# Hendrik1704/GPBayesTools-HIC

Measured on AMD Instinct MI355X. Metric: MCMC steps/s x walkers (walker log-posterior evaluations per second, whole job), higher is better.
Workload: dtype f64

## Files before the change

### gpbayestools_hic_amd/build.py

```python
import os
import subprocess
import sys

HERE = os.path.dirname(os.path.abspath(__file__))
CSRC = os.path.join(HERE, "csrc")
LIB = os.path.join(HERE, "libgpbayes.so")
LIB_DEBUG = os.path.join(HERE, "libgpbayes_debug.so")
SOURCES = ["gpb_api.hip", "gpb_fit.hip", "gpb_chol.hip", "gpb_predict.hip", "gpb_sliced.hip", "gpb_like.hip", "gpb_cov.hip", "gpb_pmap.hip", "gpb_pool.hip",
           "gpb_grad.hip", "gpb_ptlmc.hip", "gpb_smc.hip", "gpb_cv.hip"]
HEADERS = ["gpb_internal.h", "gemm_tile.h", "chol_block.h", "fast_math.h", "philox.h", os.path.join("..", "..", "include", "gpbayes.h"),
           os.path.join("..", "..", "include", "gpbayes_debug.h")]


def _stale(lib=LIB):
    if not os.path.exists(lib):
        return True
    t = os.path.getmtime(lib)
    return any(os.path.getmtime(os.path.join(CSRC, f)) > t for f in SOURCES + HEADERS)


def build_native(force=False, verbose=False, debug_variants=False):
    lib = LIB_DEBUG if debug_variants else LIB
    if not force and not _stale(lib):
        return lib
    hipcc = os.environ.get("HIPCC", "/opt/rocm/bin/hipcc")
    objs = []
    procs = []
    bdir = os.path.join(HERE, "build", "debug" if debug_variants else "product")
    os.makedirs(bdir, exist_ok=True)
    for src in SOURCES:
        obj = os.path.join(bdir, src.replace(".hip", ".o"))
        cmd = [hipcc, "--offload-arch=gfx950", "-O3", "-std=c++17", "-fPIC", "-fvisibility=hidden", "-c",
               os.path.join(CSRC, src), "-o", obj] + (["-DGPB_DEBUG_VARIANTS"] if debug_variants else [])
        if debug_variants:
            cmd += os.environ.get("GPB_DEBUG_EXTRA_DEFINES", "").split()
        if verbose:
            print(" ".join(cmd), file=sys.stderr)
        procs.append((cmd, subprocess.Popen(cmd, stdout=subprocess.PIPE, stderr=subprocess.STDOUT)))
        objs.append(obj)
    for cmd, p in procs:
        out, _ = p.communicate()
        if p.returncode != 0:
            raise RuntimeError("hipcc failed: %s\n%s" % (" ".join(cmd), out.decode()))
    cmd = [hipcc, "--offload-arch=gfx950", "-shared", "-fPIC", "-Wl,-Bsymbolic", "-o", lib] + objs + ["-ldl"]
    r = subprocess.run(cmd, stdout=subprocess.PIPE, stderr=subprocess.STDOUT)
    if r.returncode != 0:
        raise RuntimeError("link failed: %s\n%s" % (" ".join(cmd), r.stdout.decode()))
    return lib


if __name__ == "__main__":
    print(build_native(force="--force" in sys.argv, verbose=True))
    if "--debug-variants" in sys.argv:
        print(build_native(force="--force" in sys.argv, verbose=True, debug_variants=True))
```

### gpbayestools_hic_amd/csrc/gpb_sliced.hip

```cpp
#include "gpb_internal.h"

namespace gpb {

typedef int v4i __attribute__((ext_vector_type(4)));
typedef int v16i __attribute__((ext_vector_type(16)));
typedef __attribute__((address_space(3))) void* sl_lds_ptr;

template <int D>
struct SlDig {
    static constexpr int LOW = D - 1, NLEV = 2 * D - 1 - LOW, BITS = 8 * D - 1;
    static constexpr unsigned long long HALF = 0x8080808080808080ull >> (64 - 8 * D);
};
constexpr int SL_DMAX = 7;
constexpr int64_t SL_NP_MAX = 16384;
constexpr int SL_BM = 128;
template <int D, int WTN>
struct SlGeo {
    static constexpr int BN = 64 * WTN;
    static constexpr int A_CHUNKS = D * 2 * (SL_BM / 64), B_CHUNKS = D * 2 * WTN, CHUNKS = A_CHUNKS + B_CHUNKS;
    static constexpr int STAGE = CHUNKS * 1024, NSTAGE = 3;
    static constexpr int LDS = NSTAGE * STAGE + SL_BM * 8;
    static constexpr int NPW = (CHUNKS + 7) / 8, REM = CHUNKS % 8;
};
constexpr int SL_RG = 8, SL_CG = 4;
constexpr double SL_RULE = 128.0;

template <int D>
__device__ __forceinline__ unsigned long long sl_digits(long long a) {
    return ((unsigned long long)a + SlDig<D>::HALF) ^ SlDig<D>::HALF;
}

__device__ __forceinline__ int sl_exponent(double m) {
    int ex;
    const double f = frexp(m, &ex);
    return f <= 0.99 ? ex : ex + 1;
}

__global__ __launch_bounds__(256) void k_sl_rowscale(const double* __restrict__ Linv, const double* __restrict__ amp,
                                                     double* __restrict__ rowscale, int* __restrict__ rowexp,
                                                     double* __restrict__ colscale, int64_t Np, int64_t Np128) {
    const int p = blockIdx.y, lane = threadIdx.x & 63;
    const int64_t j = (int64_t)blockIdx.x * 4 + (threadIdx.x >> 6);
    if (j >= Np128) return;
    double m = 0.0;
    if (j < Np) {
        const double* row = Linv + ((int64_t)p * Np + j) * Np;
        for (int64_t k = lane; k <= j; k += 64) m = fmax(m, fabs(row[k]));
#pragma unroll
        for (int o = 32; o > 0; o >>= 1) m = fmax(m, __shfl_xor(m, o));
    }
    if (lane == 0) {
        const int e = m > 0.0 ? sl_exponent(m) : 0;
        rowexp[(int64_t)p * Np128 + j] = e;
        rowscale[(int64_t)p * Np128 + j] = ldexp(1.0, e - 14);
        if (j == 0) colscale[p] = ldexp(1.0, sl_exponent(amp[p]));
    }
}

template <int D>
__global__ __launch_bounds__(256) void k_sl_slice_linv(const double* __restrict__ Linv, const int* __restrict__ rowexp,
                                                       int8_t* __restrict__ planes, int64_t Np, int64_t Np128) {
    const int p = blockIdx.z;
    const int64_t j = (int64_t)blockIdx.x * 256 + threadIdx.x, kb = blockIdx.y;
    if (j >= Np || kb * 16 > j) return;
    const double* src = Linv + ((int64_t)p * Np + j) * Np + kb * 16;
    const int e = rowexp[(int64_t)p * Np128 + j];
    unsigned long long dg[16];
#pragma unroll
    for (int i = 0; i < 16; ++i) {
        const double x = (kb * 16 + i <= j) ? src[i] : 0.0;
        dg[i] = sl_digits<D>(__double2ll_rn(ldexp(x, SlDig<D>::BITS - e)));
    }
    const int64_t plane = (Np / 16) * Np128 * 16;
    int8_t* dst = planes + (int64_t)p * D * plane + (kb * Np128 + j) * 16;
#pragma unroll
    for (int t = 0; t < D; ++t) {
        unsigned w[4];
#pragma unroll
        for (int g = 0; g < 4; ++g)
            w[g] = (unsigned)((dg[4 * g] >> (8 * t)) & 0xff) | (unsigned)(((dg[4 * g + 1] >> (8 * t)) & 0xff) << 8) |
                   (unsigned)(((dg[4 * g + 2] >> (8 * t)) & 0xff) << 16) | (unsigned)(((dg[4 * g + 3] >> (8 * t)) & 0xff) << 24);
        *reinterpret_cast<uint4*>(dst + t * plane) = make_uint4(w[0], w[1], w[2], w[3]);
    }
}


template <int D, int WTN>
__device__ __forceinline__ void sl_dma_stage(char* lds, int buf, const int8_t* __restrict__ Ap, const int8_t* __restrict__ Bp,
                                             int64_t a_plane, int64_t b_plane, int64_t Np128, int64_t Wld, int64_t mb, int64_t nb,
                                             int64_t kb0, int wave, int lane) {
    typedef SlGeo<D, WTN> G;
    char* base = lds + buf * G::STAGE;
#pragma unroll
    for (int c = 0; c < G::NPW; ++c) {
        const int ch = 8 * c + wave;
        if (c == G::NPW - 1 && G::REM != 0 && wave >= G::REM) break;
        const bool is_a = ch < G::A_CHUNKS;
        const int cb = is_a ? ch : ch - G::A_CHUNKS;
        const int per = is_a ? SL_BM / 64 : WTN;
        const int t = cb / (2 * per), q = (cb / per) & 1, h = cb % per;
        const int64_t ld = is_a ? Np128 : Wld, off = is_a ? mb : nb;
        const int8_t* plane = is_a ? Ap + t * a_plane : Bp + t * b_plane;
        const int8_t* src = plane + ((kb0 + q) * ld + off + 64 * h + lane) * 16;
        __builtin_amdgcn_global_load_lds((const void*)src, (sl_lds_ptr)(base + ch * 1024), 16, 0, 0);
    }
}

template <int N>
__device__ __forceinline__ void sl_wait_vm() { asm volatile("s_waitcnt vmcnt(%0)" ::"n"(N) : "memory"); }

template <int D, int WTN>
__device__ __forceinline__ void sl_wait_stage(bool more, bool full_count) {
    typedef SlGeo<D, WTN> G;
    if (!more) sl_wait_vm<0>();
    else if (full_count) sl_wait_vm<G::NPW>();
    else sl_wait_vm<G::NPW - 1>();
}

template <int D, int WTN>
__device__ __forceinline__ void sl_mma_step(const char* lds, int buf, int wm, int wn, int lane, v16i (&acc)[SlDig<D>::NLEV][WTN]) {
    typedef SlGeo<D, WTN> G;
    constexpr int LOW = SlDig<D>::LOW;
    const char* base = lds + buf * G::STAGE;
    const int q = lane >> 5, r = lane & 31;
    v4i a[D];
#pragma unroll
    for (int t = 0; t < D; ++t) a[t] = *reinterpret_cast<const v4i*>(base + ((t * 2 + q) * SL_BM + wm * 32 + r) * 16);
#pragma unroll
    for (int j = 0; j < WTN; ++j) {
        v4i b[D];
#pragma unroll
        for (int t = 0; t < D; ++t)
            b[t] = *reinterpret_cast<const v4i*>(base + G::A_CHUNKS * 1024 + ((t * 2 + q) * G::BN + wn * 32 * WTN + 32 * j + r) * 16);
#pragma unroll
        for (int tb = 0; tb < D; ++tb)
#pragma unroll
            for (int ta = 0; ta < D; ++ta) {
                if (ta + tb < LOW) continue;
                acc[ta + tb - LOW][j] = __builtin_amdgcn_mfma_i32_32x32x32_i8(a[ta], b[tb], acc[ta + tb - LOW][j], 0, 0, 0);
            }
    }
}

struct SlGP {
    const int8_t *A, *B;
    const double *rowscale, *colscale;
    double* spart;
    int P, p;
};
constexpr int SL_MAX_GP = GPB_MAX_MULTI_GP;
struct SlTable { SlGP gp[SL_MAX_GP]; };

template <int D, int WTN, bool MULTI>
__device__ __forceinline__ void predict_sliced_body(const SlGP& G0, const SlTable* __restrict__ tab, int64_t Np, int64_t Np128, int64_t Wld,
                                                    int P, int nI, int nW, int kskip, const int* __restrict__ nrows) {
    typedef SlGeo<D, WTN> G;
    constexpr int NLEV = SlDig<D>::NLEV;
    extern __shared__ __attribute__((aligned(16))) char lds[];
    if (nrows) nW = (*nrows + G::BN - 1) / G::BN;
    const int nG = (nI + SL_RG - 1) / SL_RG, nWG = (nW + SL_CG - 1) / SL_CG;
    const unsigned label = blockIdx.x & 7u, m = blockIdx.x >> 3;
    const unsigned sb = (m / (SL_RG * SL_CG)) * 8u + label, local = m % (SL_RG * SL_CG);
    if (sb >= (unsigned)(nG * P * nWG)) return;
    const int g = (int)(sb / (unsigned)(P * nWG)), rem = (int)(sb % (unsigned)(P * nWG));
    const int pg = rem / nWG, wg = rem % nWG;
    const SlGP gp = MULTI ? tab->gp[pg] : G0;
    const int p = MULTI ? gp.p : pg;
    const int8_t* __restrict__ A = gp.A;
    const int8_t* __restrict__ B = gp.B;
    const double* __restrict__ rowscale = gp.rowscale;
    const double* __restrict__ colscale = gp.colscale;
    double* __restrict__ spart = gp.spart;
    const int Pc = MULTI ? gp.P : P;
    const int ib = (nG - 1 - g) * SL_RG + (SL_RG - 1 - (int)(local / SL_CG)), wt = wg * SL_CG + (int)(local % SL_CG);
    if (ib >= nI || wt >= nW) return;
    const int tid = threadIdx.x, lane = tid & 63;
    const int wave = __builtin_amdgcn_readfirstlane(tid >> 6);
    const int wm = wave >> 1, wn = wave & 1;
    const int64_t mb = (int64_t)ib * SL_BM, nb = (int64_t)wt * G::BN;
    const bool fullc = G::REM == 0 || wave < G::REM;
    const int64_t a_plane = (Np / 16) * Np128 * 16, b_plane = (Np / 16) * Wld * 16;
    const int8_t* Ap = A + (int64_t)p * D * a_plane;
    const int8_t* Bp = B + (int64_t)p * D * b_plane;
    double* rs = reinterpret_cast<double*>(lds + G::NSTAGE * G::STAGE);
    if (tid < SL_BM) rs[tid] = rowscale[(int64_t)p * Np128 + mb + tid];
    const int64_t k_end = imin64(mb + SL_BM, Np);
    const int64_t ks = (kskip / 32) * 32;
    const int64_t k_begin = ks <= mb ? ks : 0;
    const int nsteps = (int)((k_end - k_begin) / 32);
    const int64_t kb_first = k_begin / 16;
    v16i acc[NLEV][WTN];
#pragma unroll
    for (int l = 0; l < NLEV; ++l)
#pragma unroll
        for (int j = 0; j < WTN; ++j)
#pragma unroll
            for (int r = 0; r < 16; ++r) acc[l][j][r] = 0;
    sl_dma_stage<D, WTN>(lds, 0, Ap, Bp, a_plane, b_plane, Np128, Wld, mb, nb, kb_first, wave, lane);
    if (nsteps > 1) sl_dma_stage<D, WTN>(lds, 1, Ap, Bp, a_plane, b_plane, Np128, Wld, mb, nb, kb_first + 2, wave, lane);
    for (int s = 0; s < nsteps; ++s) {
        asm volatile("s_waitcnt lgkmcnt(0)" ::: "memory");
        sl_wait_stage<D, WTN>(s + 1 < nsteps, fullc);
        __builtin_amdgcn_s_barrier();
        sl_mma_step<D, WTN>(lds, s % 3, wm, wn, lane, acc);
        if (s + 2 < nsteps)
            sl_dma_stage<D, WTN>(lds, (s + 2) % 3, Ap, Bp, a_plane, b_plane, Np128, Wld, mb, nb, kb_first + 2 * (int64_t)(s + 2), wave, lane);
    }
    asm volatile("s_waitcnt lgkmcnt(0)" ::: "memory");
    __builtin_amdgcn_s_barrier();
    const double cs = colscale[p];
    double* hand = reinterpret_cast<double*>(lds);
    double sums[WTN];
#pragma unroll
    for (int j = 0; j < WTN; ++j) {
        double sum = 0.0;
#pragma unroll
        for (int r = 0; r < 16; ++r) {
            double t = (double)acc[0][j][r];
#pragma unroll
            for (int l = 1; l < NLEV; ++l) t = fma(t, 1.0 / 256.0, (double)acc[l][j][r]);
            const int row = wm * 32 + (r & 3) + 8 * (r >> 2) + 4 * (lane >> 5);
            const double v = t * rs[row] * cs;
            sum = fma(v, v, sum);
        }
        sum += __shfl_xor(sum, 32);
        sums[j] = sum;
        if ((wm & 1) && lane < 32) hand[(wave * WTN + j) * 32 + lane] = sum;
    }
    __syncthreads();
    const int64_t blk = (int64_t)ib * 2 + (wm >> 1);
    if (!(wm & 1) && lane < 32 && blk * 64 < Np) {
#pragma unroll
        for (int j = 0; j < WTN; ++j)
            spart[(blk * Pc + p) * Wld + nb + wn * 32 * WTN + 32 * j + lane] = sums[j] + hand[((wave + 2) * WTN + j) * 32 + lane];
    }
}

template <int D, int WTN>
__global__ __launch_bounds__(512, 2) void k_predict_sliced(const SlGP gp, int64_t Np, int64_t Np128, int64_t Wld, int P, int nI, int nW,
                                                           int kskip, const int* __restrict__ nrows) {
    predict_sliced_body<D, WTN, false>(gp, nullptr, Np, Np128, Wld, P, nI, nW, kskip, nrows);
}

template <int D, int WTN>
__global__ __launch_bounds__(512, 2) void k_predict_sliced_multi(const SlTable tab, int64_t Np, int64_t Np128, int64_t Wld, int P, int nI,
                                                                 int nW, int kskip, const int* __restrict__ nrows) {
    predict_sliced_body<D, WTN, true>(tab.gp[0], &tab, Np, Np128, Wld, P, nI, nW, kskip, nrows);
}

int sliced_applies(const gpb_ctx* ctx) {
    if (!ctx->predict_sliced || ctx->multi || !ctx->h_theta || !ctx->have_theta) return 0;
    if (ctx->tile_trace) return 0;
    if (ctx->Np > SL_NP_MAX) return 0;
    if (ctx->predict_sliced == 3) return 7;
    if (ctx->predict_sliced == 2) return 6;
    const int64_t stride = ctx->d + 2;
    for (int64_t p = 0; p < ctx->P; ++p) {
        const double lc = ctx->h_theta[p * stride], ln = ctx->h_theta[p * stride + ctx->d + 1];
        if (!(1.0 + exp(lc - ln) <= SL_RULE)) return 0;
    }
    return 6;
}

void sliced_free(gpb_ctx* ctx) {
    if (ctx->slA) { pool_free(ctx->slA); ctx->slA = nullptr; }
    if (ctx->slB) { pool_free(ctx->slB); ctx->slB = nullptr; }
    if (ctx->sl_scale) { pool_free(ctx->sl_scale); ctx->sl_scale = nullptr; }
    ctx->slA_valid = false;
    ctx->slA_depth = 0;
    ctx->slB_cap = 0;
}

const double* sliced_colscale(const gpb_ctx* ctx) {
    return reinterpret_cast<const double*>(ctx->sl_scale) + ctx->P * round_up(ctx->Np, 128);
}

int sliced_prepare(gpb_ctx* ctx, int depth) {
    if (depth != 6 && depth != 7) GPB_FAIL(GPB_E_STATE, "gpb: internal: sliced_prepare at a depth other than 6 or 7");
    const int64_t Np = ctx->Np, Np128 = round_up(Np, 128), P = ctx->P;
    const size_t a_bytes = (size_t)P * SL_DMAX * (size_t)Np * (size_t)Np128;
    if (!ctx->slA) {
        GPB_HIP(pool_malloc_t(&ctx->slA, a_bytes));
        GPB_HIP(hipMemsetAsync(ctx->slA, 0, a_bytes, ctx->stream));
        GPB_HIP(pool_malloc_t(&ctx->sl_scale, sizeof(double) * (size_t)(P * Np128 + P) + sizeof(int) * (size_t)(P * Np128)));
        ctx->slA_valid = false;
    }
    double* rowscale = reinterpret_cast<double*>(ctx->sl_scale);
    double* colscale = rowscale + P * Np128;
    int* rowexp = reinterpret_cast<int*>(colscale + P);
    if (!ctx->slA_valid || ctx->slA_depth != depth) {
        hipLaunchKernelGGL(k_sl_rowscale, dim3((unsigned)((Np128 + 3) / 4), (unsigned)P), dim3(256), 0, ctx->stream, ctx->Linv,
                           ctx->amp, rowscale, rowexp, colscale, Np, Np128);
        const dim3 grid((unsigned)((Np + 255) / 256), (unsigned)(Np / 16), (unsigned)P);
        if (depth == 7)
            hipLaunchKernelGGL(k_sl_slice_linv<7>, grid, dim3(256), 0, ctx->stream, ctx->Linv, rowexp, ctx->slA, Np, Np128);
        else
            hipLaunchKernelGGL(k_sl_slice_linv<6>, grid, dim3(256), 0, ctx->stream, ctx->Linv, rowexp, ctx->slA, Np, Np128);
        ctx->slA_valid = true;
        ctx->slA_depth = depth;
    }
    if (ctx->slB_cap < ctx->Wcap || !ctx->slB) {
        if (ctx->slB) { GPB_HIP(hipStreamSynchronize(ctx->stream)); pool_free(ctx->slB); ctx->slB = nullptr; }
        GPB_HIP(pool_malloc_t(&ctx->slB, (size_t)P * SL_DMAX * (size_t)Np * (size_t)ctx->Wcap));
        ctx->slB_cap = ctx->Wcap;
    }
    GPB_HIP(hipGetLastError());
    return 0;
}

int sliced_read_kstar(gpb_ctx* ctx, int64_t p, int64_t pad, int64_t N, int64_t W, double* out) {
    const int D = ctx->batch_sliced;
    if (D != 6 && D != 7) GPB_FAIL(GPB_E_STATE, "gpb: internal: sliced_read_kstar without a sliced batch");
    const int64_t Np = ctx->Np, Wld = ctx->Wld, plane = (Np / 16) * Wld * 16;
    std::vector<int8_t> h((size_t)(D * plane));
    double cs = 0.0;
    GPB_HIP(hipStreamSynchronize(ctx->stream));
    GPB_HIP(hipMemcpy(h.data(), ctx->slB + p * D * plane, (size_t)(D * plane), hipMemcpyDeviceToHost));
    GPB_HIP(hipMemcpy(&cs, sliced_colscale(ctx) + p, sizeof(double), hipMemcpyDeviceToHost));
    for (int64_t n = 0; n < N; ++n)
        for (int64_t w = 0; w < W; ++w) {
            const int64_t k = pad + n;
            long long a = 0;
            for (int t = D - 1; t >= 0; --t) a = a * 256 + (long long)h[(size_t)(t * plane + ((k / 16) * Wld + w) * 16 + k % 16)];
            out[n * W + w] = ldexp((double)a, -(8 * D - 1)) * cs;
        }
    return 0;
}

static int sliced_wtn(const gpb_ctx* ctx, int depth, int64_t gps, int nI, int64_t W, const int* nrows_dev) {
    if (depth == 7) return 1;
    const int64_t Wsel = imin64(ctx->Wld, live_rows_estimate(ctx, W, nrows_dev, ctx->Wld));
    const int64_t tiles128 = gps * nI * ((Wsel + 127) / 128);
    int wtn = tiles128 >= 3 * (int64_t)ctx->num_cu ? 2 : 1;
    if (ctx->force_tile == 128) wtn = 2;
    if (ctx->force_tile == 64 || ctx->force_tile == 32 || ctx->force_tile == 65) wtn = 1;
    return wtn;
}

template <int D, int WTN, bool MULTI, class Arg>
static int sliced_launch(gpb_ctx* ctx, const Arg& arg, int64_t Np, int64_t Np128, int64_t Wld, int G, int nI, int kskip,
                         const int* nrows_dev) {
    typedef SlGeo<D, WTN> Geo;
    const int nW = (int)(Wld / Geo::BN);
    const int nG = (nI + SL_RG - 1) / SL_RG, nWG = (nW + SL_CG - 1) / SL_CG;
    const int64_t nSB = (int64_t)nG * G * nWG;
    const unsigned grid = (unsigned)(((nSB + 7) / 8) * 8 * SL_RG * SL_CG);
    if constexpr (MULTI) {
        GPB_HIP(hipFuncSetAttribute((const void*)k_predict_sliced_multi<D, WTN>, hipFuncAttributeMaxDynamicSharedMemorySize, Geo::LDS));
        hipLaunchKernelGGL((k_predict_sliced_multi<D, WTN>), dim3(grid), dim3(512), Geo::LDS, ctx->stream, arg, Np, Np128, Wld, G, nI, nW,
                           kskip, nrows_dev);
    } else {
        GPB_HIP(hipFuncSetAttribute((const void*)k_predict_sliced<D, WTN>, hipFuncAttributeMaxDynamicSharedMemorySize, Geo::LDS));
        hipLaunchKernelGGL((k_predict_sliced<D, WTN>), dim3(grid), dim3(512), Geo::LDS, ctx->stream, arg, Np, Np128, Wld, G, nI, nW,
                           kskip, nrows_dev);
    }
    return 0;
}

template <bool MULTI, class Arg>
static int sliced_dispatch(gpb_ctx* ctx, int depth, int wtn, const Arg& arg, int64_t Np, int64_t Np128, int64_t Wld, int G, int nI,
                           int kskip, const int* nrows_dev) {
    if (depth == 7) return sliced_launch<7, 1, MULTI>(ctx, arg, Np, Np128, Wld, G, nI, kskip, nrows_dev);
    if (wtn == 2) return sliced_launch<6, 2, MULTI>(ctx, arg, Np, Np128, Wld, G, nI, kskip, nrows_dev);
    return sliced_launch<6, 1, MULTI>(ctx, arg, Np, Np128, Wld, G, nI, kskip, nrows_dev);
}

int launch_vsq_sliced(gpb_ctx* ctx, int64_t W, const int* nrows_dev, int kskip) {
    const int64_t Np = ctx->Np, Np128 = round_up(Np, 128), P = ctx->P, Wld = ctx->Wld;
    const int depth = ctx->batch_sliced;
    if (!ctx->slA || !ctx->slA_valid || !ctx->slB || ctx->slA_depth != depth)
        GPB_FAIL(GPB_E_STATE, "gpb: internal: launch_vsq_sliced before sliced_prepare");
    const double* rowscale = reinterpret_cast<const double*>(ctx->sl_scale);
    const double* colscale = rowscale + P * Np128;
    const int nI = (int)(Np128 / SL_BM);
    const int wtn = sliced_wtn(ctx, depth, P, nI, W, nrows_dev);
    const SlGP gp{ctx->slA, ctx->slB, rowscale, colscale, ctx->spart, (int)P, 0};
    return sliced_dispatch<false>(ctx, depth, wtn, gp, Np, Np128, Wld, (int)P, nI, kskip, nrows_dev);
}

int launch_vsq_sliced_multi(gpb_ctx* const* ctxs, int E, int64_t W, const int* nrows_dev, int kskip) {
    gpb_ctx* ctx = ctxs[0];
    const int64_t Np = ctx->Np, Np128 = round_up(Np, 128), Wld = ctx->Wld;
    const int depth = ctx->batch_sliced;
    SlTable tab;
    int G = 0;
    for (int e = 0; e < E; ++e) {
        gpb_ctx* c = ctxs[e];
        if (!c->slA || !c->slA_valid || !c->slB || c->Np != Np || c->Wld != Wld || c->batch_sliced != depth || c->slA_depth != depth)
            GPB_FAIL(GPB_E_STATE, "gpb: internal: launch_vsq_sliced_multi over a context that is not prepared");
        const double* rowscale = reinterpret_cast<const double*>(c->sl_scale);
        const double* colscale = rowscale + c->P * Np128;
        for (int p = 0; p < (int)c->P; ++p, ++G) {
            if (G >= SL_MAX_GP) GPB_FAIL(GPB_E_STATE, "gpb: internal: launch_vsq_sliced_multi: too many GPs for one table");
            tab.gp[G] = SlGP{c->slA, c->slB, rowscale, colscale, c->spart, (int)c->P, p};
        }
    }
    const int nI = (int)(Np128 / SL_BM);
    const int wtn = sliced_wtn(ctx, depth, G, nI, W, nrows_dev);
    return sliced_dispatch<true>(ctx, depth, wtn, tab, Np, Np128, Wld, G, nI, kskip, nrows_dev);
}

}
```

Baseline: 1.497 million.

## Ping-pong wave groups between LDS reads and MFMA in sliced GEMM

Replaces the per-step read-then-MFMA loop with a schedule in which two groups of four waves alternate between loading LDS operands and issuing MFMAs. The group offset comes from one extra barrier, so one group's LDS reads overlap the other group's matrix work, and each step is split into per-column sub-steps. The DMA source address is also made wave-uniform through readfirstlane, with the lane offset added afterwards. The cost is roughly twice as many barriers per step plus extra sched_barrier fences that limit compiler reordering.

```diff
diff --git a/gpbayestools_hic_amd/build.py b/gpbayestools_hic_amd/build.py
--- a/gpbayestools_hic_amd/build.py
+++ b/gpbayestools_hic_amd/build.py
@@ -8,7 +8,7 @@
 LIB_DEBUG = os.path.join(HERE, "libgpbayes_debug.so")
 SOURCES = ["gpb_api.hip", "gpb_fit.hip", "gpb_chol.hip", "gpb_predict.hip", "gpb_sliced.hip", "gpb_like.hip", "gpb_cov.hip", "gpb_pmap.hip", "gpb_pool.hip",
            "gpb_grad.hip", "gpb_ptlmc.hip", "gpb_smc.hip", "gpb_cv.hip"]
-HEADERS = ["gpb_internal.h", "gemm_tile.h", "chol_block.h", "fast_math.h", "philox.h", os.path.join("..", "..", "include", "gpbayes.h"),
+HEADERS = ["gpb_internal.h", "gemm_tile.h", "sliced_schedule.h", "chol_block.h", "fast_math.h", "philox.h", os.path.join("..", "..", "include", "gpbayes.h"),
            os.path.join("..", "..", "include", "gpbayes_debug.h")]
 
 
diff --git a/gpbayestools_hic_amd/csrc/gpb_sliced.hip b/gpbayestools_hic_amd/csrc/gpb_sliced.hip
--- a/gpbayestools_hic_amd/csrc/gpb_sliced.hip
+++ b/gpbayestools_hic_amd/csrc/gpb_sliced.hip
@@ -1,4 +1,5 @@
 #include "gpb_internal.h"
+#include "sliced_schedule.h"
 
 namespace gpb {
 
@@ -21,6 +22,8 @@
     static constexpr int STAGE = CHUNKS * 1024, NSTAGE = 3;
     static constexpr int LDS = NSTAGE * STAGE + SL_BM * 8;
     static constexpr int NPW = (CHUNKS + 7) / 8, REM = CHUNKS % 8;
+    static_assert(NSTAGE == SL_SCHED_BUFFERS && CHUNKS == sl_sched_chunks(D, WTN) && NPW == sl_sched_npw(D, WTN) && REM == sl_sched_rem(D, WTN),
+                  "sliced_schedule.h models another geometry");
 };
 constexpr int SL_RG = 8, SL_CG = 4;
 constexpr double SL_RULE = 128.0;
@@ -101,8 +104,10 @@
         const int t = cb / (2 * per), q = (cb / per) & 1, h = cb % per;
         const int64_t ld = is_a ? Np128 : Wld, off = is_a ? mb : nb;
         const int8_t* plane = is_a ? Ap + t * a_plane : Bp + t * b_plane;
-        const int8_t* src = plane + ((kb0 + q) * ld + off + 64 * h + lane) * 16;
-        __builtin_amdgcn_global_load_lds((const void*)src, (sl_lds_ptr)(base + ch * 1024), 16, 0, 0);
+        const uint64_t us = (uint64_t)(plane + ((kb0 + q) * ld + off + 64 * h) * 16);
+        const int8_t* src = (const int8_t*)(((uint64_t)(unsigned)__builtin_amdgcn_readfirstlane((int)(us >> 32)) << 32) |
+                                            (uint64_t)(unsigned)__builtin_amdgcn_readfirstlane((int)us));
+        __builtin_amdgcn_global_load_lds((const void*)(src + (unsigned)(lane << 4)), (sl_lds_ptr)(base + ch * 1024), 16, 0, 0);
     }
 }
 
@@ -118,29 +123,51 @@
 }
 
 template <int D, int WTN>
-__device__ __forceinline__ void sl_mma_step(const char* lds, int buf, int wm, int wn, int lane, v16i (&acc)[SlDig<D>::NLEV][WTN]) {
+struct SlWave {
     typedef SlGeo<D, WTN> G;
-    constexpr int LOW = SlDig<D>::LOW;
-    const char* base = lds + buf * G::STAGE;
-    const int q = lane >> 5, r = lane & 31;
-    v4i a[D];
-#pragma unroll
-    for (int t = 0; t < D; ++t) a[t] = *reinterpret_cast<const v4i*>(base + ((t * 2 + q) * SL_BM + wm * 32 + r) * 16);
-#pragma unroll
-    for (int j = 0; j < WTN; ++j) {
-        v4i b[D];
-#pragma unroll
-        for (int t = 0; t < D; ++t)
-            b[t] = *reinterpret_cast<const v4i*>(base + G::A_CHUNKS * 1024 + ((t * 2 + q) * G::BN + wn * 32 * WTN + 32 * j + r) * 16);
+    static constexpr int NLEV = SlDig<D>::NLEV, LOW = SlDig<D>::LOW;
+    char* lds;
+    const int8_t *Ap, *Bp;
+    int64_t a_plane, b_plane, Np128, Wld, mb, nb, kb_first;
+    int wave, lane, wm, wn;
+    bool fullc;
+    v4i a[D], b[D];
+    v16i acc[NLEV][WTN];
+
+    __device__ __forceinline__ void issue(int stage, int buf) {
+        sl_dma_stage<D, WTN>(lds, buf, Ap, Bp, a_plane, b_plane, Np128, Wld, mb, nb, kb_first + 2 * (int64_t)stage, wave, lane);
+    }
+    template <int J>
+    __device__ __forceinline__ void read(int, int buf) {
+        const int q = lane >> 5, r = lane & 31;
+        const char* pa = lds + (buf * G::STAGE + (q * SL_BM + wm * 32 + r) * 16);
+        const char* pb = lds + (buf * G::STAGE + G::A_CHUNKS * 1024 + (q * G::BN + wn * 32 * WTN + r) * 16);
+#pragma unroll
+        for (int t = 0; t < D; ++t) a[t] = *reinterpret_cast<const v4i*>(pa + t * 2 * SL_BM * 16);
+#pragma unroll
+        for (int t = 0; t < D; ++t) b[t] = *reinterpret_cast<const v4i*>(pb + (t * 2 * G::BN + 32 * J) * 16);
+    }
+    __device__ __forceinline__ void reads_done() { asm volatile("s_waitcnt lgkmcnt(0)" ::: "memory"); }
+    __device__ __forceinline__ void wait(bool newest_flies) {
+        reads_done();
+        sl_wait_stage<D, WTN>(newest_flies, fullc);
+    }
+    __device__ __forceinline__ void barrier() {
+        __builtin_amdgcn_sched_barrier(0);
+        __builtin_amdgcn_s_barrier();
+        __builtin_amdgcn_sched_barrier(0);
+    }
+    template <int J>
+    __device__ __forceinline__ void mma() {
 #pragma unroll
         for (int tb = 0; tb < D; ++tb)
 #pragma unroll
             for (int ta = 0; ta < D; ++ta) {
                 if (ta + tb < LOW) continue;
-                acc[ta + tb - LOW][j] = __builtin_amdgcn_mfma_i32_32x32x32_i8(a[ta], b[tb], acc[ta + tb - LOW][j], 0, 0, 0);
+                acc[ta + tb - LOW][J] = __builtin_amdgcn_mfma_i32_32x32x32_i8(a[ta], b[tb], acc[ta + tb - LOW][J], 0, 0, 0);
             }
     }
-}
+};
 
 struct SlGP {
     const int8_t *A, *B;
@@ -189,25 +216,16 @@
     const int64_t k_begin = ks <= mb ? ks : 0;
     const int nsteps = (int)((k_end - k_begin) / 32);
     const int64_t kb_first = k_begin / 16;
-    v16i acc[NLEV][WTN];
+    SlWave<D, WTN> w;
+    w.lds = lds; w.Ap = Ap; w.Bp = Bp; w.a_plane = a_plane; w.b_plane = b_plane; w.Np128 = Np128; w.Wld = Wld;
+    w.mb = mb; w.nb = nb; w.kb_first = kb_first; w.wave = wave; w.lane = lane; w.wm = wm; w.wn = wn; w.fullc = fullc;
 #pragma unroll
     for (int l = 0; l < NLEV; ++l)
 #pragma unroll
         for (int j = 0; j < WTN; ++j)
 #pragma unroll
-            for (int r = 0; r < 16; ++r) acc[l][j][r] = 0;
-    sl_dma_stage<D, WTN>(lds, 0, Ap, Bp, a_plane, b_plane, Np128, Wld, mb, nb, kb_first, wave, lane);
-    if (nsteps > 1) sl_dma_stage<D, WTN>(lds, 1, Ap, Bp, a_plane, b_plane, Np128, Wld, mb, nb, kb_first + 2, wave, lane);
-    for (int s = 0; s < nsteps; ++s) {
-        asm volatile("s_waitcnt lgkmcnt(0)" ::: "memory");
-        sl_wait_stage<D, WTN>(s + 1 < nsteps, fullc);
-        __builtin_amdgcn_s_barrier();
-        sl_mma_step<D, WTN>(lds, s % 3, wm, wn, lane, acc);
-        if (s + 2 < nsteps)
-            sl_dma_stage<D, WTN>(lds, (s + 2) % 3, Ap, Bp, a_plane, b_plane, Np128, Wld, mb, nb, kb_first + 2 * (int64_t)(s + 2), wave, lane);
-    }
-    asm volatile("s_waitcnt lgkmcnt(0)" ::: "memory");
-    __builtin_amdgcn_s_barrier();
+            for (int r = 0; r < 16; ++r) w.acc[l][j][r] = 0;
+    sl_sched_walk<WTN>(wave >> 2, nsteps, w);
     const double cs = colscale[p];
     double* hand = reinterpret_cast<double*>(lds);
     double sums[WTN];
@@ -216,9 +234,9 @@
         double sum = 0.0;
 #pragma unroll
         for (int r = 0; r < 16; ++r) {
-            double t = (double)acc[0][j][r];
-#pragma unroll
-            for (int l = 1; l < NLEV; ++l) t = fma(t, 1.0 / 256.0, (double)acc[l][j][r]);
+            double t = (double)w.acc[0][j][r];
+#pragma unroll
+            for (int l = 1; l < NLEV; ++l) t = fma(t, 1.0 / 256.0, (double)w.acc[l][j][r]);
             const int row = wm * 32 + (r & 3) + 8 * (r >> 2) + 4 * (lane >> 5);
             const double v = t * rs[row] * cs;
             sum = fma(v, v, sum);
diff --git a/gpbayestools_hic_amd/csrc/sliced_schedule.h b/gpbayestools_hic_amd/csrc/sliced_schedule.h
--- /dev/null
+++ b/gpbayestools_hic_amd/csrc/sliced_schedule.h
@@ -0,0 +1,80 @@
+#ifndef GPB_SLICED_SCHEDULE_H
+#define GPB_SLICED_SCHEDULE_H
+
+#if defined(__HIPCC__) || defined(__CUDACC__)
+#define SL_HD __host__ __device__ __forceinline__
+#else
+#define SL_HD inline
+#endif
+
+constexpr int SL_SCHED_BUFFERS = 3;
+constexpr int SL_SCHED_WAVES = 8;
+
+constexpr int sl_sched_chunks(int D, int WTN) { return D * 2 * 2 + D * 2 * WTN; }
+constexpr int sl_sched_npw(int D, int WTN) { return (sl_sched_chunks(D, WTN) + SL_SCHED_WAVES - 1) / SL_SCHED_WAVES; }
+constexpr int sl_sched_rem(int D, int WTN) { return sl_sched_chunks(D, WTN) % SL_SCHED_WAVES; }
+constexpr int sl_sched_wave_dmas(int wave, int D, int WTN) {
+    return (sl_sched_rem(D, WTN) == 0 || wave < sl_sched_rem(D, WTN)) ? sl_sched_npw(D, WTN) : sl_sched_npw(D, WTN) - 1;
+}
+constexpr int sl_sched_vmcnt(bool newest_flies, int wave_dmas) { return newest_flies ? wave_dmas : 0; }
+
+constexpr int sl_sched_substeps(int nsteps, int JS) { return nsteps * JS; }
+constexpr int sl_sched_halfsteps(int nsteps, int JS) { return 2 * nsteps * JS + 1; }
+constexpr int sl_sched_barriers(int nsteps, int JS) { return sl_sched_halfsteps(nsteps, JS) + 1; }
+constexpr int sl_sched_load_halfstep(int g, int v) { return 2 * v + g; }
+constexpr int sl_sched_mma_halfstep(int g, int v) { return 2 * v + g + 1; }
+constexpr int sl_sched_buffer(int stage) { return stage % SL_SCHED_BUFFERS; }
+
+enum SlRole { SL_IDLE = 0, SL_LOAD = 1, SL_MMA = 2 };
+
+struct SlHalfStep {
+    int role, v, j;
+    int read_stage, read_buf;
+    int issue_stage, issue_buf;
+    int wait_stage;
+    bool newest_flies;
+};
+
+SL_HD SlHalfStep sl_sched_at(int g, int h, int nsteps, int JS) {
+    SlHalfStep e = {SL_IDLE, -1, -1, -1, -1, -1, -1, -1, false};
+    const int nv = nsteps * JS, t = h - g;
+    if (t < 0 || t >= 2 * nv) return e;
+    e.v = t / 2;
+    e.j = e.v % JS;
+    const int s = e.v / JS;
+    if (t & 1) { e.role = SL_MMA; return e; }
+    e.role = SL_LOAD;
+    e.read_stage = s;
+    e.read_buf = sl_sched_buffer(s);
+    if (e.j == 0 && s + 2 < nsteps) { e.issue_stage = s + 2; e.issue_buf = sl_sched_buffer(s + 2); }
+    if (e.j == JS - 1) {
+        if (s + 1 < nsteps) e.wait_stage = s + 1;
+        e.newest_flies = s + 2 < nsteps;
+    }
+    return e;
+}
+
+template <int JS, int J, class V>
+SL_HD void sl_sched_substep(int s, int nsteps, V& vis) {
+    vis.template read<J>(s, sl_sched_buffer(s));
+    if (J == 0 && s + 2 < nsteps) vis.issue(s + 2, sl_sched_buffer(s + 2));
+    if (J == JS - 1) vis.wait(s + 2 < nsteps);
+    else vis.reads_done();
+    vis.barrier();
+    vis.template mma<J>();
+    vis.barrier();
+    if constexpr (J + 1 < JS) sl_sched_substep<JS, J + 1>(s, nsteps, vis);
+}
+
+template <int JS, class V>
+SL_HD void sl_sched_walk(int g, int nsteps, V& vis) {
+    vis.issue(0, sl_sched_buffer(0));
+    if (nsteps > 1) vis.issue(1, sl_sched_buffer(1));
+    vis.wait(nsteps > 1);
+    vis.barrier();
+    if (g == 1) vis.barrier();
+    for (int s = 0; s < nsteps; ++s) sl_sched_substep<JS, 0>(s, nsteps, vis);
+    if (g == 0) vis.barrier();
+}
+
+#endif
```

New measurement: 1.499 million (median of 5 runs). No clear change (+0.1%).
